# tyfeld/MMaDA-Parallel

Hardware: NVIDIA H100
Metric: denoised_tokens_per_sec (higher is better)
Workload: dtype bf16; 1 GPU; MMaDA-Parallel-A 8B, 1 prompt per GPU, 512x512 (1024 VQ tokens) + 256 text tokens, timesteps=64, text_steps=128, cfg_img=4.0, cfg_scale=0, temperature=1.0, text_temperature=0 (BASELINE configs[1]); seq_len=2414, parallelism=replicas x1 (independent prompts, no collective), weights=synthetic normal(0, 0.02) bf16, seeded, l2=16.2 GB of weights streamed per forward >> 50 MB L2 (no flush needed)

## Files before the change

mmada_parallel_b200/csrc/attention.cu:

```cuda
#include "mmdp_internal.h"
#include "ptx.cuh"

#include <stdlib.h>

#include <map>
#include <mutex>
#include <utility>

namespace mmdp {

static constexpr int kAttnThreads = 384;
static constexpr int kQBytes = 128 * 128 * 2;
template <int BKV> struct AttnCfg {
    static constexpr int kKBytes = BKV * 128 * 2;
    static constexpr int kVBytes = 128 * BKV * 2;
    static constexpr int kSmem = kQBytes + 2 * (kKBytes + kVBytes) + 1024  + 256 ;
};

__device__ __forceinline__ float ex2_approx(float x) {
    float y;
    asm("ex2.approx.ftz.f32 %0, %1;" : "=f"(y) : "f"(x));
    return y;
}

struct AttnSegs {
    int n;
    int start[kMaxSegs + 1];
    int tile0[kMaxSegs + 1];
};

struct AttnWin {
    AttnSegs segs;
    int q0[kMaxSegs], nq[kMaxSegs], out0[kMaxSegs];
};

template <int kBKV, bool kPacked, bool kGqa = false, bool kWin = false>
__device__ __forceinline__ void attention_body(const CUtensorMap& tmQ, const CUtensorMap& tmK, const CUtensorMap& tmVt,
                                               __nv_bfloat16* __restrict__ out, int H, int L, int d_model, float scale_log2,
                                               int n_full, int splits, float* __restrict__ part_ws, int Lq, const AttnSegs* segs,
                                               int kv_group = 1, const AttnWin* win = nullptr) {
    constexpr int kKBytes = AttnCfg<kBKV>::kKBytes, kVBytes = AttnCfg<kBKV>::kVBytes;
    extern __shared__ uint8_t smem_raw[];
    uint8_t* smem = reinterpret_cast<uint8_t*>((reinterpret_cast<uintptr_t>(smem_raw) + 1023) & ~uintptr_t(1023));
    uint8_t* sQ = smem;
    uint8_t* sK = sQ + kQBytes;
    uint8_t* sV = sK + 2 * kKBytes;
    uint64_t* bars = reinterpret_cast<uint64_t*>(sV + 2 * kVBytes);
    uint64_t* q_full = bars + 0;
    uint64_t* k_full = bars + 1;
    uint64_t* k_empty = bars + 3;
    uint64_t* v_full = bars + 5;
    uint64_t* v_empty = bars + 7;

    const int warp = threadIdx.x >> 5, lane = threadIdx.x & 31, wg = warp >> 2;
    int n_qt = (Lq + 127) / 128;
    int n_kv_all = (L + kBKV - 1) / kBKV;
    int tile = blockIdx.x, piece = -1;
    if ((int)blockIdx.x >= n_full) {
        const int t = (int)blockIdx.x - n_full;
        tile = n_full + t / splits;
        piece = t - (t / splits) * splits;
    }
    int seg = 0, seg0 = 0, tl = tile, q0 = 0, o0 = 0;
    if constexpr (kPacked) {
        for (int i = 1; i < segs->n; ++i)
            if (tile >= segs->tile0[i]) seg = i;
        seg0 = segs->start[seg];
        L = Lq = segs->start[seg + 1] - seg0;
        o0 = seg0;
        if constexpr (kWin) {
            q0 = win->q0[seg];
            Lq = win->nq[seg];
            o0 = win->out0[seg];
        }
        n_qt = (Lq + 127) / 128;
        n_kv_all = (L + kBKV - 1) / kBKV;
        tl = tile - segs->tile0[seg];
    }
    const int qt = tl % n_qt, h = (tl / n_qt) % H, b = kPacked ? seg : tile / (n_qt * H);
    const int hk = kGqa ? h / kv_group : h, Hk = kGqa ? H / kv_group : H;
    int jb = 0, je = n_kv_all;
    if (piece >= 0) {
        const int per = (n_kv_all + splits - 1) / splits;
        jb = piece * per;
        je = (jb + per < n_kv_all) ? jb + per : n_kv_all;
    }
    const int n_kv = je - jb;

    if (warp == 0 && lane == 0) {
        tma_prefetch_desc(&tmQ);
        tma_prefetch_desc(&tmK);
        tma_prefetch_desc(&tmVt);
        mbar_init(q_full, 1);
        for (int s = 0; s < 2; ++s) {
            mbar_init(&k_full[s], 1);
            mbar_init(&k_empty[s], 8);
            mbar_init(&v_full[s], 1);
            mbar_init(&v_empty[s], 8);
        }
        fence_barrier_init();
    }
    __syncthreads();
    pdl_launch_dependents();
    pdl_wait();

    if (wg == 0) {
        setmaxnreg_dec<40>();
        if (warp == 0 && elect_one_sync()) {
            const int qrow0 = (kPacked ? seg0 + q0 : b * Lq) + qt * 128;
            mbar_expect_tx(q_full, kQBytes);
            tma_load_2d(sQ, &tmQ, q_full, h * 128, qrow0);
            tma_load_2d(sQ + kQBytes / 2, &tmQ, q_full, h * 128 + 64, qrow0);
            for (int j = 0; j < n_kv; ++j) {
                const int st = j & 1;
                const uint32_t ph = (j >> 1) & 1;
                const int kv0 = (jb + j) * kBKV;
                mbar_wait(&k_empty[st], ph ^ 1);
                mbar_expect_tx(&k_full[st], kKBytes);
                tma_load_2d(sK + st * kKBytes, &tmK, &k_full[st], hk * 128, (kPacked ? seg0 : b * L) + kv0);
                tma_load_2d(sK + st * kKBytes + kKBytes / 2, &tmK, &k_full[st], hk * 128 + 64, (kPacked ? seg0 : b * L) + kv0);
                mbar_wait(&v_empty[st], ph ^ 1);
                mbar_expect_tx(&v_full[st], kVBytes);
                tma_load_2d(sV + st * kVBytes, &tmVt, &v_full[st], kv0, (b * Hk + hk) * 128);
                if (kBKV == 128) tma_load_2d(sV + st * kVBytes + kVBytes / 2, &tmVt, &v_full[st], kv0 + 64, (b * Hk + hk) * 128);
            }
        }
        __syncwarp();
        return;
    }

    setmaxnreg_inc<232>();
    const int half = wg - 1;
    const int r0 = half * 64 + (warp & 3) * 16 + (lane >> 2), c0 = 2 * (lane & 3);
    const uint32_t aQ = smem_u32(sQ) + half * (64 * 128);
    float o[64];
#pragma unroll
    for (int i = 0; i < 64; ++i) o[i] = 0.f;
    float m_run[2] = {-INFINITY, -INFINITY}, l_run[2] = {0.f, 0.f};
    mbar_wait(q_full, 0);
    for (int j = 0; j < n_kv; ++j) {
        const int st = j & 1;
        const uint32_t ph = (j >> 1) & 1;
        const int nvalid = L - (jb + j) * kBKV;
        float sacc[kBKV / 2];
        const uint32_t aK = smem_u32(sK + st * kKBytes);
        mbar_wait(&k_full[st], ph);
        wgmma_fence();
#pragma unroll
        for (int kk = 0; kk < 8; ++kk)
        {
            const uint64_t qd = smem_desc_kmajor_sw128(aQ + (kk >> 2) * (kQBytes / 2)) + (kk & 3) * 2;
            const uint64_t kd = smem_desc_kmajor_sw128(aK + (kk >> 2) * (kKBytes / 2)) + (kk & 3) * 2;
            if constexpr (kBKV == 128) wgmma_bf16_ss_n128(sacc, qd, kd, kk != 0);
            else wgmma_bf16_ss_n64(sacc, qd, kd, kk != 0);
        }
        wgmma_commit();
        wgmma_wait<0>();
        reg_fence(sacc);
        __syncwarp();
        if (lane == 0) mbar_arrive(&k_empty[st]);
        if (nvalid < kBKV) {
#pragma unroll
            for (int jj = 0; jj < kBKV / 8; ++jj)
#pragma unroll
                for (int e = 0; e < 2; ++e)
                    if (8 * jj + c0 + e >= nvalid) { sacc[4 * jj + e] = -INFINITY; sacc[4 * jj + 2 + e] = -INFINITY; }
        }
        float alpha[2], mneg[2];
#pragma unroll
        for (int hh = 0; hh < 2; ++hh) {
            float mx = sacc[2 * hh];
#pragma unroll
            for (int jj = 0; jj < kBKV / 8; ++jj) mx = fmaxf(mx, fmaxf(sacc[4 * jj + 2 * hh], sacc[4 * jj + 2 * hh + 1]));
            mx = fmaxf(mx, __shfl_xor_sync(0xffffffffu, mx, 1));
            mx = fmaxf(mx, __shfl_xor_sync(0xffffffffu, mx, 2));
            const float m_new = fmaxf(m_run[hh], mx);
            alpha[hh] = ex2_approx((m_run[hh] - m_new) * scale_log2);
            m_run[hh] = m_new;
            mneg[hh] = -m_new * scale_log2;
        }
        uint32_t pa[kBKV / 4];
        float rsum[2] = {0.f, 0.f};
#pragma unroll
        for (int jj = 0; jj < kBKV / 8; ++jj)
#pragma unroll
            for (int hh = 0; hh < 2; ++hh) {
                const float p0 = ex2_approx(fmaf(sacc[4 * jj + 2 * hh], scale_log2, mneg[hh]));
                const float p1 = ex2_approx(fmaf(sacc[4 * jj + 2 * hh + 1], scale_log2, mneg[hh]));
                rsum[hh] += p0 + p1;
                pa[2 * jj + hh] = pack_bf16x2(p0, p1);
            }
#pragma unroll
        for (int hh = 0; hh < 2; ++hh) l_run[hh] = fmaf(l_run[hh], alpha[hh], rsum[hh]);
#pragma unroll
        for (int jj = 0; jj < 16; ++jj) {
            o[4 * jj] *= alpha[0]; o[4 * jj + 1] *= alpha[0];
            o[4 * jj + 2] *= alpha[1]; o[4 * jj + 3] *= alpha[1];
        }
        const uint32_t aV = smem_u32(sV + st * kVBytes);
        mbar_wait(&v_full[st], ph);
        wgmma_fence();
#pragma unroll
        for (int kk = 0; kk < kBKV / 16; ++kk) {
            const uint32_t a[4] = {pa[4 * kk], pa[4 * kk + 1], pa[4 * kk + 2], pa[4 * kk + 3]};
            wgmma_bf16_rs_n128(o, a, smem_desc_kmajor_sw128(aV + (kk >> 2) * (kVBytes / 2)) + (kk & 3) * 2, 1);
        }
        wgmma_commit();
        wgmma_wait<0>();
        reg_fence(o);
        __syncwarp();
        if (lane == 0) mbar_arrive(&v_empty[st]);
    }
#pragma unroll
    for (int hh = 0; hh < 2; ++hh) {
        l_run[hh] += __shfl_xor_sync(0xffffffffu, l_run[hh], 1);
        l_run[hh] += __shfl_xor_sync(0xffffffffu, l_run[hh], 2);
    }
#pragma unroll
    for (int hh = 0; hh < 2; ++hh) {
        const int r = r0 + 8 * hh, qrow = qt * 128 + r;
        if (qrow >= Lq) continue;
        if (piece >= 0) {
            float* slot = part_ws + (size_t)((tile - n_full) * splits + piece) * (128 * 128 + 256);
            if ((lane & 3) == 0) {
                slot[128 * 128 + r] = m_run[hh];
                slot[128 * 128 + 128 + r] = l_run[hh];
            }
#pragma unroll
            for (int jj = 0; jj < 16; ++jj)
                *reinterpret_cast<float2*>(slot + (size_t)r * 128 + 8 * jj + c0) = make_float2(o[4 * jj + 2 * hh], o[4 * jj + 2 * hh + 1]);
        } else {
            const float inv_l = 1.0f / l_run[hh];
            __nv_bfloat16* orow = out + (size_t)((kPacked ? o0 : b * Lq) + qrow) * d_model + h * 128;
#pragma unroll
            for (int jj = 0; jj < 16; ++jj)
                *reinterpret_cast<uint32_t*>(orow + 8 * jj + c0) = pack_bf16x2(o[4 * jj + 2 * hh] * inv_l, o[4 * jj + 2 * hh + 1] * inv_l);
        }
    }
}

template <int kBKV>
__global__ void __launch_bounds__(kAttnThreads, 1)
attention_kernel(const __grid_constant__ CUtensorMap tmQ, const __grid_constant__ CUtensorMap tmK,
                 const __grid_constant__ CUtensorMap tmVt, __nv_bfloat16* __restrict__ out, int H, int L, int d_model,
                 float scale_log2, int n_full, int splits, float* __restrict__ part_ws, int Lq) {
    attention_body<kBKV, false>(tmQ, tmK, tmVt, out, H, L, d_model, scale_log2, n_full, splits, part_ws, Lq, nullptr);
}

template <int kBKV>
__global__ void __launch_bounds__(kAttnThreads, 1)
attention_packed_kernel(const __grid_constant__ CUtensorMap tmQ, const __grid_constant__ CUtensorMap tmK,
                        const __grid_constant__ CUtensorMap tmVt, __nv_bfloat16* __restrict__ out, int H, int d_model,
                        float scale_log2, int n_full, int splits, float* __restrict__ part_ws, const __grid_constant__ AttnSegs segs) {
    attention_body<kBKV, true>(tmQ, tmK, tmVt, out, H, 0, d_model, scale_log2, n_full, splits, part_ws, 0, &segs);
}

template <int kBKV>
__global__ void __launch_bounds__(kAttnThreads, 1)
attention_gqa_kernel(const __grid_constant__ CUtensorMap tmQ, const __grid_constant__ CUtensorMap tmK,
                     const __grid_constant__ CUtensorMap tmVt, __nv_bfloat16* __restrict__ out, int H, int L, int d_model,
                     float scale_log2, int n_full, int splits, float* __restrict__ part_ws, int Lq, int kv_group) {
    attention_body<kBKV, false, true>(tmQ, tmK, tmVt, out, H, L, d_model, scale_log2, n_full, splits, part_ws, Lq, nullptr, kv_group);
}

template <int kBKV>
__global__ void __launch_bounds__(kAttnThreads, 1)
attention_packed_gqa_kernel(const __grid_constant__ CUtensorMap tmQ, const __grid_constant__ CUtensorMap tmK,
                            const __grid_constant__ CUtensorMap tmVt, __nv_bfloat16* __restrict__ out, int H, int d_model,
                            float scale_log2, int n_full, int splits, float* __restrict__ part_ws, const __grid_constant__ AttnSegs segs,
                            int kv_group) {
    attention_body<kBKV, true, true>(tmQ, tmK, tmVt, out, H, 0, d_model, scale_log2, n_full, splits, part_ws, 0, &segs, kv_group);
}

template <int kBKV, bool kGqa>
__global__ void __launch_bounds__(kAttnThreads, 1)
attention_packed_window_kernel(const __grid_constant__ CUtensorMap tmQ, const __grid_constant__ CUtensorMap tmK,
                               const __grid_constant__ CUtensorMap tmVt, __nv_bfloat16* __restrict__ out, int H, int d_model,
                               float scale_log2, int n_full, int splits, float* __restrict__ part_ws, const __grid_constant__ AttnWin win,
                               int kv_group) {
    attention_body<kBKV, true, kGqa, true>(tmQ, tmK, tmVt, out, H, 0, d_model, scale_log2, n_full, splits, part_ws, 0, &win.segs,
                                           kv_group, &win);
}

template <bool kPacked, bool kWin = false>
__device__ __forceinline__ void attention_combine_body(const float* __restrict__ part_ws, __nv_bfloat16* __restrict__ out, int H,
                                                       int Lq, int d_model, float scale_log2, int n_full, int splits,
                                                       const AttnSegs* segs, const AttnWin* win = nullptr) {
    int n_qt = (Lq + 127) / 128;
    const int st = blockIdx.x, r = blockIdx.y, c = threadIdx.x;
    pdl_launch_dependents();
    pdl_wait();
    const int tile = n_full + st;
    int seg = 0, seg0 = 0, tl = tile;
    if constexpr (kPacked) {
        for (int i = 1; i < segs->n; ++i)
            if (tile >= segs->tile0[i]) seg = i;
        seg0 = segs->start[seg];
        Lq = segs->start[seg + 1] - seg0;
        if constexpr (kWin) {
            seg0 = win->out0[seg];
            Lq = win->nq[seg];
        }
        n_qt = (Lq + 127) / 128;
        tl = tile - segs->tile0[seg];
    }
    const int qt = tl % n_qt, h = (tl / n_qt) % H, b = kPacked ? seg : tile / (n_qt * H);
    const int qrow = qt * 128 + r;
    if (qrow >= Lq) return;
    const float* base = part_ws + (size_t)st * splits * (128 * 128 + 256);
    float m = -INFINITY;
    for (int i = 0; i < splits; ++i) m = fmaxf(m, base[(size_t)i * (128 * 128 + 256) + 128 * 128 + r]);
    float o = 0.f, l = 0.f;
    for (int i = 0; i < splits; ++i) {
        const float* slot = base + (size_t)i * (128 * 128 + 256);
        const float w = exp2f((slot[128 * 128 + r] - m) * scale_log2);
        o = fmaf(w, slot[(size_t)r * 128 + c], o);
        l = fmaf(w, slot[128 * 128 + 128 + r], l);
    }
    out[(size_t)((kPacked ? seg0 : b * Lq) + qrow) * d_model + h * 128 + c] = __float2bfloat16_rn(o / l);
}

__global__ void __launch_bounds__(128)
attention_combine_kernel(const float* __restrict__ part_ws, __nv_bfloat16* __restrict__ out, int H, int Lq, int d_model,
                         float scale_log2, int n_full, int splits) {
    attention_combine_body<false>(part_ws, out, H, Lq, d_model, scale_log2, n_full, splits, nullptr);
}

__global__ void __launch_bounds__(128)
attention_packed_combine_kernel(const float* __restrict__ part_ws, __nv_bfloat16* __restrict__ out, int H, int d_model,
                                float scale_log2, int n_full, int splits, const __grid_constant__ AttnSegs segs) {
    attention_combine_body<true>(part_ws, out, H, 0, d_model, scale_log2, n_full, splits, &segs);
}

__global__ void __launch_bounds__(128)
attention_packed_window_combine_kernel(const float* __restrict__ part_ws, __nv_bfloat16* __restrict__ out, int H, int d_model,
                                       float scale_log2, int n_full, int splits, const __grid_constant__ AttnWin win) {
    attention_combine_body<true, true>(part_ws, out, H, 0, d_model, scale_log2, n_full, splits, &win.segs, &win);
}

static std::map<std::pair<int, cudaStream_t>, std::pair<float*, size_t>> g_attn_ws;
static std::mutex g_attn_ws_mu;
static int attn_part_workspace(cudaStream_t stream, size_t need, float** out) {
    int dev = 0;
    MMDP_CUDA(cudaGetDevice(&dev));
    std::lock_guard<std::mutex> lk(g_attn_ws_mu);
    auto& e = g_attn_ws[std::make_pair(dev, stream)];
    if (need > e.second) {
        if (e.first) MMDP_CUDA(cudaFree(e.first));
        e.first = nullptr; e.second = 0;
        MMDP_CUDA(cudaMalloc(&e.first, need));
        e.second = need;
    }
    *out = e.first;
    return 0;
}

template <class KvbOf>
static void plan_split_tail(int tiles, KvbOf kvb_of, int& n_full, int& n_split, int& splits) {
    const int split_tail = opt(OPT_ATTN_SPLIT_TAIL), slots = num_sms();
    n_full = tiles; n_split = 0; splits = 1;
    auto fit_splits = [&](int want, int first) {
        int sp = want > 8 ? 8 : want;
        for (int t = first; t < tiles; ++t)
            if (sp > kvb_of(t) / 2) sp = kvb_of(t) / 2;
        auto empty_piece = [&](int s) {
            for (int t = first; t < tiles; ++t) {
                const int n_kvb = kvb_of(t);
                if ((s - 1) * ((n_kvb + s - 1) / s) >= n_kvb) return true;
            }
            return false;
        };
        while (sp >= 2 && empty_piece(sp)) --sp;
        return sp;
    };
    if (split_tail && tiles > slots && (tiles % slots) > 0 && (tiles % slots) * 4 <= slots) {
        n_split = tiles % slots;
        splits = fit_splits(slots / n_split, tiles - n_split);
        if (splits >= 2) n_full = tiles - n_split; else { n_split = 0; splits = 1; }
    } else if (split_tail && tiles * 2 <= slots) {
        splits = fit_splits(slots / tiles, 0);
        if (splits >= 2) { n_split = tiles; n_full = 0; } else splits = 1;
    }
}

template <class Kernel>
static int attn_smem_attr(Kernel kernel, int smem, unsigned long long& attr_set) {
    int dev = 0;
    MMDP_CUDA(cudaGetDevice(&dev));
    if (!(attr_set >> (dev & 63) & 1ull)) {
        MMDP_CUDA(cudaFuncSetAttribute(kernel, cudaFuncAttributeMaxDynamicSharedMemorySize, smem));
        attr_set |= 1ull << (dev & 63);
    }
    return 0;
}

template <int kBKV>
static int attention_launch(const __nv_bfloat16* q, const __nv_bfloat16* k, const __nv_bfloat16* vt, __nv_bfloat16* out, int B, int H,
                            int L, int Lpad, float scale, cudaStream_t stream, int Lq, int Hkv) {
    constexpr int kAttnSmem = AttnCfg<kBKV>::kSmem;
    if (B <= 0 || H <= 0 || L <= 0) return set_error("attention: empty problem");
    if (Lq <= 0) Lq = L;
    if (Hkv <= 0) Hkv = H;
    if (Hkv > H || H % Hkv) return set_error("attention: n_kv_heads=%d must divide n_heads=%d", Hkv, H);
    if (Lpad < L || (Lpad % 8)) return set_error("attention: Lpad must be >= L and a multiple of 8");
    const int d_model = H * 128, d_kv = Hkv * 128;
    CUtensorMap tmQ, tmK, tmVt;
    if (make_tmap_2d_bf16(&tmQ, q, (uint64_t)B * Lq, (uint64_t)d_model, (uint64_t)d_model, 128, 64)) return -1;
    if (make_tmap_2d_bf16(&tmK, k, (uint64_t)B * L, (uint64_t)d_kv, (uint64_t)d_kv, kBKV, 64)) return -1;
    if (make_tmap_2d_bf16(&tmVt, vt, (uint64_t)B * Hkv * 128, (uint64_t)Lpad, (uint64_t)Lpad, 128, 64)) return -1;
    const int n_qt = (Lq + 127) / 128, n_kvb = (L + kBKV - 1) / kBKV;
    const int tiles = n_qt * H * B;
    int n_full, n_split, splits;
    plan_split_tail(tiles, [&](int) { return n_kvb; }, n_full, n_split, splits);
    float* part_ws = nullptr;
    if (n_split > 0 && attn_part_workspace(stream, (size_t)n_split * splits * (128 * 128 + 256) * sizeof(float), &part_ws)) return -1;
    const int grid = n_full + n_split * splits;
    const float scale_log2 = scale * 1.4426950408889634f;
    const bool pdl = pdl_mode() != 0;
    LaunchScope ls(LK_ATTN, 4.0 * B * H * (double)Lq * L * 128, stream);
    if (Hkv != H) {
        static unsigned long long attr_set_gqa = 0;
        if (attn_smem_attr(attention_gqa_kernel<kBKV>, kAttnSmem, attr_set_gqa)) return -1;
        MMDP_CUDA(launch_ex(attention_gqa_kernel<kBKV>, dim3(grid), dim3(kAttnThreads), kAttnSmem, stream, pdl, false, tmQ, tmK, tmVt, out,
                            H, L, d_model, scale_log2, n_full, splits, part_ws, Lq, H / Hkv));
    } else {
        static unsigned long long attr_set = 0;
        if (attn_smem_attr(attention_kernel<kBKV>, kAttnSmem, attr_set)) return -1;
        MMDP_CUDA(launch_ex(attention_kernel<kBKV>, dim3(grid), dim3(kAttnThreads), kAttnSmem, stream, pdl, false, tmQ, tmK, tmVt, out, H, L,
                            d_model, scale_log2, n_full, splits, part_ws, Lq));
    }
    if (n_split > 0)
        MMDP_CUDA(launch_ex(attention_combine_kernel, dim3(n_split, 128), dim3(128), 0, stream, pdl, false, (const float*)part_ws, out, H, Lq,
                            d_model, scale_log2, n_full, splits));
    return 0;
}

template <int kBKV>
static int attention_packed_launch(const __nv_bfloat16* q, const __nv_bfloat16* k, const __nv_bfloat16* vt, __nv_bfloat16* out,
                                   const SegTable& segs, int H, int Lpad, float scale, cudaStream_t stream, int Hkv,
                                   const int* win_lo, const int* win_hi) {
    constexpr int kAttnSmem = AttnCfg<kBKV>::kSmem;
    if (segs.n <= 0 || segs.n > kMaxSegs || H <= 0) return set_error("attention_packed: %d sequences (1 to %d)", segs.n, kMaxSegs);
    if (Hkv <= 0) Hkv = H;
    if (Hkv > H || H % Hkv) return set_error("attention_packed: n_kv_heads=%d must divide n_heads=%d", Hkv, H);
    if (Lpad % 8) return set_error("attention_packed: Lpad must be a multiple of 8");
    if (!win_lo != !win_hi) return set_error("attention_packed: give both window bounds or neither");
    const bool windowed = win_lo != nullptr;
    AttnWin aw{};
    AttnSegs& as = aw.segs;
    as.n = segs.n;
    double work = 0;
    int Mq = 0;
    for (int s = 0; s <= segs.n; ++s) {
        as.start[s] = segs.start[s];
        if (s == segs.n) break;
        const int len = segs.start[s + 1] - segs.start[s];
        if (len <= 0 || len > Lpad) return set_error("attention_packed: sequence %d has length %d (Lpad %d)", s, len, Lpad);
        const int lo = windowed ? win_lo[s] : 0, hi = windowed ? win_hi[s] : len;
        if (lo < 0 || lo >= hi || hi > len)
            return set_error("attention_packed: sequence %d of length %d has the row window [%d, %d)", s, len, lo, hi);
        aw.q0[s] = lo;
        aw.nq[s] = hi - lo;
        aw.out0[s] = Mq;
        Mq += hi - lo;
        as.tile0[s + 1] = as.tile0[s] + (hi - lo + 127) / 128 * H;
        work += 4.0 * H * (double)(hi - lo) * len * 128;
    }
    const int M = segs.start[segs.n], tiles = as.tile0[segs.n], d_model = H * 128, d_kv = Hkv * 128;
    CUtensorMap tmQ, tmK, tmVt;
    if (make_tmap_2d_bf16(&tmQ, q, (uint64_t)M, (uint64_t)d_model, (uint64_t)d_model, 128, 64)) return -1;
    if (make_tmap_2d_bf16(&tmK, k, (uint64_t)M, (uint64_t)d_kv, (uint64_t)d_kv, kBKV, 64)) return -1;
    if (make_tmap_2d_bf16(&tmVt, vt, (uint64_t)segs.n * Hkv * 128, (uint64_t)Lpad, (uint64_t)Lpad, 128, 64)) return -1;
    auto kvb_of = [&](int t) {
        int s = 0;
        while (s + 1 < segs.n && t >= as.tile0[s + 1]) ++s;
        return (segs.start[s + 1] - segs.start[s] + kBKV - 1) / kBKV;
    };
    int n_full, n_split, splits;
    plan_split_tail(tiles, kvb_of, n_full, n_split, splits);
    float* part_ws = nullptr;
    if (n_split > 0 && attn_part_workspace(stream, (size_t)n_split * splits * (128 * 128 + 256) * sizeof(float), &part_ws)) return -1;
    const int grid = n_full + n_split * splits;
    const float scale_log2 = scale * 1.4426950408889634f;
    const bool pdl = pdl_mode() != 0;
    LaunchScope ls(LK_ATTN, work, stream);
    if (windowed) {
        auto kernel = Hkv != H ? attention_packed_window_kernel<kBKV, true> : attention_packed_window_kernel<kBKV, false>;
        static unsigned long long attr_set_win[2] = {0, 0};
        if (attn_smem_attr(kernel, kAttnSmem, attr_set_win[Hkv != H])) return -1;
        MMDP_CUDA(launch_ex(kernel, dim3(grid), dim3(kAttnThreads), kAttnSmem, stream, pdl, false, tmQ, tmK, tmVt, out, H, d_model,
                            scale_log2, n_full, splits, part_ws, aw, H / Hkv));
        if (n_split > 0)
            MMDP_CUDA(launch_ex(attention_packed_window_combine_kernel, dim3(n_split, 128), dim3(128), 0, stream, pdl, false,
                                (const float*)part_ws, out, H, d_model, scale_log2, n_full, splits, aw));
        return 0;
    }
    if (Hkv != H) {
        static unsigned long long attr_set_gqa = 0;
        if (attn_smem_attr(attention_packed_gqa_kernel<kBKV>, kAttnSmem, attr_set_gqa)) return -1;
        MMDP_CUDA(launch_ex(attention_packed_gqa_kernel<kBKV>, dim3(grid), dim3(kAttnThreads), kAttnSmem, stream, pdl, false, tmQ, tmK, tmVt,
                            out, H, d_model, scale_log2, n_full, splits, part_ws, as, H / Hkv));
    } else {
        static unsigned long long attr_set = 0;
        if (attn_smem_attr(attention_packed_kernel<kBKV>, kAttnSmem, attr_set)) return -1;
        MMDP_CUDA(launch_ex(attention_packed_kernel<kBKV>, dim3(grid), dim3(kAttnThreads), kAttnSmem, stream, pdl, false, tmQ, tmK, tmVt, out,
                            H, d_model, scale_log2, n_full, splits, part_ws, as));
    }
    if (n_split > 0)
        MMDP_CUDA(launch_ex(attention_packed_combine_kernel, dim3(n_split, 128), dim3(128), 0, stream, pdl, false, (const float*)part_ws,
                            out, H, d_model, scale_log2, n_full, splits, as));
    return 0;
}

int attention_fwd(const __nv_bfloat16* q, const __nv_bfloat16* k, const __nv_bfloat16* vt, __nv_bfloat16* out, int B, int H, int L,
                  int Lpad, float scale, cudaStream_t stream, int Lq, int Hkv) {
// ... 17 lines not shown
```

mmada_parallel_b200/csrc/ptx.cuh:

```cuda
#pragma once
#include <cuda.h>
#include <cuda_bf16.h>
#include <cuda_runtime.h>
#include <stdint.h>

namespace mmdp {

__device__ __forceinline__ uint32_t smem_u32(const void* p) {
    return static_cast<uint32_t>(__cvta_generic_to_shared(p));
}

__device__ __forceinline__ bool elect_one_sync() {
    uint32_t pred;
    asm volatile(
        "{\n\t.reg .pred p;\n\t"
        "elect.sync _|p, 0xffffffff;\n\t"
        "selp.u32 %0, 1, 0, p;\n\t}"
        : "=r"(pred));
    return pred != 0;
}

#ifndef MMDP_WAIT_SPIN_LIMIT
#define MMDP_WAIT_SPIN_LIMIT (1u << 26)
#endif

__device__ __forceinline__ void mbar_init(uint64_t* bar, uint32_t count) {
    asm volatile("mbarrier.init.shared::cta.b64 [%0], %1;" ::"r"(smem_u32(bar)), "r"(count));
}
__device__ __forceinline__ void fence_barrier_init() {
    asm volatile("fence.mbarrier_init.release.cluster;" ::: "memory");
}
__device__ __forceinline__ void mbar_expect_tx(uint64_t* bar, uint32_t bytes) {
    asm volatile("mbarrier.arrive.expect_tx.shared::cta.b64 _, [%0], %1;" ::"r"(smem_u32(bar)), "r"(bytes)
                 : "memory");
}
__device__ __forceinline__ void mbar_arrive(uint64_t* bar) {
    asm volatile("mbarrier.arrive.shared::cta.b64 _, [%0];" ::"r"(smem_u32(bar)) : "memory");
}
__device__ __forceinline__ bool mbar_try_wait(uint64_t* bar, uint32_t parity) {
    uint32_t ok;
    asm volatile(
        "{\n\t.reg .pred p;\n\t"
        "mbarrier.try_wait.parity.shared::cta.b64 p, [%1], %2;\n\t"
        "selp.b32 %0, 1, 0, p;\n\t}"
        : "=r"(ok)
        : "r"(smem_u32(bar)), "r"(parity)
        : "memory");
    return ok != 0;
}
__device__ __forceinline__ void mbar_wait(uint64_t* bar, uint32_t parity) {
    uint32_t spins = 0;
    while (!mbar_try_wait(bar, parity)) {
        if (++spins > MMDP_WAIT_SPIN_LIMIT) __trap();
    }
}

__device__ __forceinline__ void fence_proxy_async_smem() {
    asm volatile("fence.proxy.async.shared::cta;" ::: "memory");
}

__device__ __forceinline__ void tma_prefetch_desc(const CUtensorMap* tm) {
    asm volatile("prefetch.tensormap [%0];" ::"l"(reinterpret_cast<uint64_t>(tm)) : "memory");
}
__device__ __forceinline__ void tma_load_2d(void* smem_dst, const CUtensorMap* tm, uint64_t* bar, int c0, int c1) {
    asm volatile(
        "cp.async.bulk.tensor.2d.shared::cluster.global.mbarrier::complete_tx::bytes [%0], [%1, {%3, %4}], [%2];"
        ::"r"(smem_u32(smem_dst)), "l"(reinterpret_cast<uint64_t>(tm)), "r"(smem_u32(bar)), "r"(c0), "r"(c1)
        : "memory");
}

__device__ __forceinline__ void tma_load_2d_multicast(void* smem_dst, const CUtensorMap* tm, uint64_t* bar, int c0, int c1,
                                                      uint16_t cta_mask) {
    asm volatile(
        "cp.async.bulk.tensor.2d.shared::cluster.global.mbarrier::complete_tx::bytes.multicast::cluster [%0], [%1, {%3, %4}], [%2], %5;"
        ::"r"(smem_u32(smem_dst)), "l"(reinterpret_cast<uint64_t>(tm)), "r"(smem_u32(bar)), "r"(c0), "r"(c1), "h"(cta_mask)
        : "memory");
}

__device__ __forceinline__ uint32_t cluster_ctarank() {
    uint32_t r;
    asm volatile("mov.u32 %0, %%cluster_ctarank;" : "=r"(r));
    return r;
}
__device__ __forceinline__ void cluster_sync() {
    asm volatile("barrier.cluster.arrive.release.aligned;\n\tbarrier.cluster.wait.acquire.aligned;" ::: "memory");
}
__device__ __forceinline__ void mbar_arrive_cluster(uint64_t* bar, uint32_t cta) {
    asm volatile(
        "{\n\t.reg .b32 ra;\n\t"
        "mapa.shared::cluster.u32 ra, %0, %1;\n\t"
        "mbarrier.arrive.release.cluster.shared::cluster.b64 _, [ra];\n\t}"
        ::"r"(smem_u32(bar)), "r"(cta)
        : "memory");
}

__device__ __forceinline__ void tma_prefetch_l2_2d(const CUtensorMap* tm, int c0, int c1) {
    asm volatile("cp.async.bulk.prefetch.tensor.2d.L2.global.tile [%0, {%1, %2}];" ::"l"(reinterpret_cast<uint64_t>(tm)),
                 "r"(c0), "r"(c1)
                 : "memory");
}

__device__ __forceinline__ void pdl_wait() { asm volatile("griddepcontrol.wait;" ::: "memory"); }
__device__ __forceinline__ void pdl_launch_dependents() { asm volatile("griddepcontrol.launch_dependents;" ::: "memory"); }

__device__ __forceinline__ void wgmma_fence() { asm volatile("wgmma.fence.sync.aligned;" ::: "memory"); }
__device__ __forceinline__ void wgmma_commit() { asm volatile("wgmma.commit_group.sync.aligned;" ::: "memory"); }
template <int N>
__device__ __forceinline__ void wgmma_wait() { asm volatile("wgmma.wait_group.sync.aligned %0;" ::"n"(N) : "memory"); }
template <int N>
__device__ __forceinline__ void reg_fence(float (&d)[N]) {
#pragma unroll
    for (int i = 0; i < N; ++i) asm volatile("" : "+f"(d[i])::"memory");
}
template <uint32_t kRegs>
__device__ __forceinline__ void setmaxnreg_dec() { asm volatile("setmaxnreg.dec.sync.aligned.u32 %0;" ::"n"(kRegs)); }
template <uint32_t kRegs>
__device__ __forceinline__ void setmaxnreg_inc() { asm volatile("setmaxnreg.inc.sync.aligned.u32 %0;" ::"n"(kRegs)); }

__device__ __forceinline__ void wgmma_bf16_ss_n256(float (&d)[128], uint64_t a_desc, uint64_t b_desc, int scale_d) {
    asm volatile(
        "{\n\t.reg .pred p;\n\t"
        "setp.ne.b32 p, %130, 0;\n\t"
        "wgmma.mma_async.sync.aligned.m64n256k16.f32.bf16.bf16 "
        "{%0, %1, %2, %3, %4, %5, %6, %7, %8, %9, %10, %11, %12, %13, %14, %15, %16, %17, %18, %19, %20, %21, %22, %23, %24, %25, %26, %27, %28, %29, %30, %31, %32, %33, %34, %35, %36, %37, %38, %39, %40, %41, %42, %43, %44, %45, %46, %47, %48, %49, %50, %51, %52, %53, %54, %55, %56, %57, %58, %59, %60, %61, %62, %63, %64, %65, %66, %67, %68, %69, %70, %71, %72, %73, %74, %75, %76, %77, %78, %79, %80, %81, %82, %83, %84, %85, %86, %87, %88, %89, %90, %91, %92, %93, %94, %95, %96, %97, %98, %99, %100, %101, %102, %103, %104, %105, %106, %107, %108, %109, %110, %111, %112, %113, %114, %115, %116, %117, %118, %119, %120, %121, %122, %123, %124, %125, %126, %127}, "
        "%128, %129, p, 1, 1, 0, 0;\n\t}"
        : "+f"(d[0]), "+f"(d[1]), "+f"(d[2]), "+f"(d[3]), "+f"(d[4]), "+f"(d[5]), "+f"(d[6]), "+f"(d[7]), "+f"(d[8]), "+f"(d[9]), "+f"(d[10]), "+f"(d[11]), "+f"(d[12]), "+f"(d[13]), "+f"(d[14]), "+f"(d[15]), "+f"(d[16]), "+f"(d[17]), "+f"(d[18]), "+f"(d[19]), "+f"(d[20]), "+f"(d[21]), "+f"(d[22]), "+f"(d[23]), "+f"(d[24]), "+f"(d[25]), "+f"(d[26]), "+f"(d[27]), "+f"(d[28]), "+f"(d[29]), "+f"(d[30]), "+f"(d[31]), "+f"(d[32]), "+f"(d[33]), "+f"(d[34]), "+f"(d[35]), "+f"(d[36]), "+f"(d[37]), "+f"(d[38]), "+f"(d[39]), "+f"(d[40]), "+f"(d[41]), "+f"(d[42]), "+f"(d[43]), "+f"(d[44]), "+f"(d[45]), "+f"(d[46]), "+f"(d[47]), "+f"(d[48]), "+f"(d[49]), "+f"(d[50]), "+f"(d[51]), "+f"(d[52]), "+f"(d[53]), "+f"(d[54]), "+f"(d[55]), "+f"(d[56]), "+f"(d[57]), "+f"(d[58]), "+f"(d[59]), "+f"(d[60]), "+f"(d[61]), "+f"(d[62]), "+f"(d[63]), "+f"(d[64]), "+f"(d[65]), "+f"(d[66]), "+f"(d[67]), "+f"(d[68]), "+f"(d[69]), "+f"(d[70]), "+f"(d[71]), "+f"(d[72]), "+f"(d[73]), "+f"(d[74]), "+f"(d[75]), "+f"(d[76]), "+f"(d[77]), "+f"(d[78]), "+f"(d[79]), "+f"(d[80]), "+f"(d[81]), "+f"(d[82]), "+f"(d[83]), "+f"(d[84]), "+f"(d[85]), "+f"(d[86]), "+f"(d[87]), "+f"(d[88]), "+f"(d[89]), "+f"(d[90]), "+f"(d[91]), "+f"(d[92]), "+f"(d[93]), "+f"(d[94]), "+f"(d[95]), "+f"(d[96]), "+f"(d[97]), "+f"(d[98]), "+f"(d[99]), "+f"(d[100]), "+f"(d[101]), "+f"(d[102]), "+f"(d[103]), "+f"(d[104]), "+f"(d[105]), "+f"(d[106]), "+f"(d[107]), "+f"(d[108]), "+f"(d[109]), "+f"(d[110]), "+f"(d[111]), "+f"(d[112]), "+f"(d[113]), "+f"(d[114]), "+f"(d[115]), "+f"(d[116]), "+f"(d[117]), "+f"(d[118]), "+f"(d[119]), "+f"(d[120]), "+f"(d[121]), "+f"(d[122]), "+f"(d[123]), "+f"(d[124]), "+f"(d[125]), "+f"(d[126]), "+f"(d[127])
        : "l"(a_desc), "l"(b_desc), "r"(scale_d));
}

__device__ __forceinline__ void wgmma_bf16_ss_n192(float (&d)[96], uint64_t a_desc, uint64_t b_desc, int scale_d) {
    asm volatile(
        "{\n\t.reg .pred p;\n\t"
        "setp.ne.b32 p, %98, 0;\n\t"
        "wgmma.mma_async.sync.aligned.m64n192k16.f32.bf16.bf16 "
        "{%0, %1, %2, %3, %4, %5, %6, %7, %8, %9, %10, %11, %12, %13, %14, %15, %16, %17, %18, %19, %20, %21, %22, %23, %24, %25, %26, %27, %28, %29, %30, %31, %32, %33, %34, %35, %36, %37, %38, %39, %40, %41, %42, %43, %44, %45, %46, %47, %48, %49, %50, %51, %52, %53, %54, %55, %56, %57, %58, %59, %60, %61, %62, %63, %64, %65, %66, %67, %68, %69, %70, %71, %72, %73, %74, %75, %76, %77, %78, %79, %80, %81, %82, %83, %84, %85, %86, %87, %88, %89, %90, %91, %92, %93, %94, %95}, "
        "%96, %97, p, 1, 1, 0, 0;\n\t}"
        : "+f"(d[0]), "+f"(d[1]), "+f"(d[2]), "+f"(d[3]), "+f"(d[4]), "+f"(d[5]), "+f"(d[6]), "+f"(d[7]), "+f"(d[8]), "+f"(d[9]), "+f"(d[10]), "+f"(d[11]), "+f"(d[12]), "+f"(d[13]), "+f"(d[14]), "+f"(d[15]), "+f"(d[16]), "+f"(d[17]), "+f"(d[18]), "+f"(d[19]), "+f"(d[20]), "+f"(d[21]), "+f"(d[22]), "+f"(d[23]), "+f"(d[24]), "+f"(d[25]), "+f"(d[26]), "+f"(d[27]), "+f"(d[28]), "+f"(d[29]), "+f"(d[30]), "+f"(d[31]), "+f"(d[32]), "+f"(d[33]), "+f"(d[34]), "+f"(d[35]), "+f"(d[36]), "+f"(d[37]), "+f"(d[38]), "+f"(d[39]), "+f"(d[40]), "+f"(d[41]), "+f"(d[42]), "+f"(d[43]), "+f"(d[44]), "+f"(d[45]), "+f"(d[46]), "+f"(d[47]), "+f"(d[48]), "+f"(d[49]), "+f"(d[50]), "+f"(d[51]), "+f"(d[52]), "+f"(d[53]), "+f"(d[54]), "+f"(d[55]), "+f"(d[56]), "+f"(d[57]), "+f"(d[58]), "+f"(d[59]), "+f"(d[60]), "+f"(d[61]), "+f"(d[62]), "+f"(d[63]), "+f"(d[64]), "+f"(d[65]), "+f"(d[66]), "+f"(d[67]), "+f"(d[68]), "+f"(d[69]), "+f"(d[70]), "+f"(d[71]), "+f"(d[72]), "+f"(d[73]), "+f"(d[74]), "+f"(d[75]), "+f"(d[76]), "+f"(d[77]), "+f"(d[78]), "+f"(d[79]), "+f"(d[80]), "+f"(d[81]), "+f"(d[82]), "+f"(d[83]), "+f"(d[84]), "+f"(d[85]), "+f"(d[86]), "+f"(d[87]), "+f"(d[88]), "+f"(d[89]), "+f"(d[90]), "+f"(d[91]), "+f"(d[92]), "+f"(d[93]), "+f"(d[94]), "+f"(d[95])
        : "l"(a_desc), "l"(b_desc), "r"(scale_d));
}

__device__ __forceinline__ void wgmma_bf16_ss_n128(float (&d)[64], uint64_t a_desc, uint64_t b_desc, int scale_d) {
    asm volatile(
        "{\n\t.reg .pred p;\n\t"
        "setp.ne.b32 p, %66, 0;\n\t"
        "wgmma.mma_async.sync.aligned.m64n128k16.f32.bf16.bf16 "
        "{%0, %1, %2, %3, %4, %5, %6, %7, %8, %9, %10, %11, %12, %13, %14, %15, %16, %17, %18, %19, %20, %21, %22, %23, %24, %25, %26, %27, %28, %29, %30, %31, %32, %33, %34, %35, %36, %37, %38, %39, %40, %41, %42, %43, %44, %45, %46, %47, %48, %49, %50, %51, %52, %53, %54, %55, %56, %57, %58, %59, %60, %61, %62, %63}, "
        "%64, %65, p, 1, 1, 0, 0;\n\t}"
        : "+f"(d[0]), "+f"(d[1]), "+f"(d[2]), "+f"(d[3]), "+f"(d[4]), "+f"(d[5]), "+f"(d[6]), "+f"(d[7]), "+f"(d[8]), "+f"(d[9]), "+f"(d[10]), "+f"(d[11]), "+f"(d[12]), "+f"(d[13]), "+f"(d[14]), "+f"(d[15]), "+f"(d[16]), "+f"(d[17]), "+f"(d[18]), "+f"(d[19]), "+f"(d[20]), "+f"(d[21]), "+f"(d[22]), "+f"(d[23]), "+f"(d[24]), "+f"(d[25]), "+f"(d[26]), "+f"(d[27]), "+f"(d[28]), "+f"(d[29]), "+f"(d[30]), "+f"(d[31]), "+f"(d[32]), "+f"(d[33]), "+f"(d[34]), "+f"(d[35]), "+f"(d[36]), "+f"(d[37]), "+f"(d[38]), "+f"(d[39]), "+f"(d[40]), "+f"(d[41]), "+f"(d[42]), "+f"(d[43]), "+f"(d[44]), "+f"(d[45]), "+f"(d[46]), "+f"(d[47]), "+f"(d[48]), "+f"(d[49]), "+f"(d[50]), "+f"(d[51]), "+f"(d[52]), "+f"(d[53]), "+f"(d[54]), "+f"(d[55]), "+f"(d[56]), "+f"(d[57]), "+f"(d[58]), "+f"(d[59]), "+f"(d[60]), "+f"(d[61]), "+f"(d[62]), "+f"(d[63])
        : "l"(a_desc), "l"(b_desc), "r"(scale_d));
}

__device__ __forceinline__ void wgmma_bf16_ss_n64(float (&d)[32], uint64_t a_desc, uint64_t b_desc, int scale_d) {
    asm volatile(
        "{\n\t.reg .pred p;\n\t"
        "setp.ne.b32 p, %34, 0;\n\t"
        "wgmma.mma_async.sync.aligned.m64n64k16.f32.bf16.bf16 "
        "{%0, %1, %2, %3, %4, %5, %6, %7, %8, %9, %10, %11, %12, %13, %14, %15, %16, %17, %18, %19, %20, %21, %22, %23, %24, %25, %26, %27, %28, %29, %30, %31}, "
        "%32, %33, p, 1, 1, 0, 0;\n\t}"
        : "+f"(d[0]), "+f"(d[1]), "+f"(d[2]), "+f"(d[3]), "+f"(d[4]), "+f"(d[5]), "+f"(d[6]), "+f"(d[7]), "+f"(d[8]), "+f"(d[9]), "+f"(d[10]), "+f"(d[11]), "+f"(d[12]), "+f"(d[13]), "+f"(d[14]), "+f"(d[15]), "+f"(d[16]), "+f"(d[17]), "+f"(d[18]), "+f"(d[19]), "+f"(d[20]), "+f"(d[21]), "+f"(d[22]), "+f"(d[23]), "+f"(d[24]), "+f"(d[25]), "+f"(d[26]), "+f"(d[27]), "+f"(d[28]), "+f"(d[29]), "+f"(d[30]), "+f"(d[31])
        : "l"(a_desc), "l"(b_desc), "r"(scale_d));
}

__device__ __forceinline__ void wgmma_bf16_rs_n128(float (&d)[64], const uint32_t (&a)[4], uint64_t b_desc, int scale_d) {
    asm volatile(
        "{\n\t.reg .pred p;\n\t"
        "setp.ne.b32 p, %69, 0;\n\t"
        "wgmma.mma_async.sync.aligned.m64n128k16.f32.bf16.bf16 "
        "{%0, %1, %2, %3, %4, %5, %6, %7, %8, %9, %10, %11, %12, %13, %14, %15, %16, %17, %18, %19, %20, %21, %22, %23, %24, %25, %26, %27, %28, %29, %30, %31, %32, %33, %34, %35, %36, %37, %38, %39, %40, %41, %42, %43, %44, %45, %46, %47, %48, %49, %50, %51, %52, %53, %54, %55, %56, %57, %58, %59, %60, %61, %62, %63}, "
        "{%64, %65, %66, %67}, %68, p, 1, 1, 0;\n\t}"
        : "+f"(d[0]), "+f"(d[1]), "+f"(d[2]), "+f"(d[3]), "+f"(d[4]), "+f"(d[5]), "+f"(d[6]), "+f"(d[7]), "+f"(d[8]), "+f"(d[9]), "+f"(d[10]), "+f"(d[11]), "+f"(d[12]), "+f"(d[13]), "+f"(d[14]), "+f"(d[15]), "+f"(d[16]), "+f"(d[17]), "+f"(d[18]), "+f"(d[19]), "+f"(d[20]), "+f"(d[21]), "+f"(d[22]), "+f"(d[23]), "+f"(d[24]), "+f"(d[25]), "+f"(d[26]), "+f"(d[27]), "+f"(d[28]), "+f"(d[29]), "+f"(d[30]), "+f"(d[31]), "+f"(d[32]), "+f"(d[33]), "+f"(d[34]), "+f"(d[35]), "+f"(d[36]), "+f"(d[37]), "+f"(d[38]), "+f"(d[39]), "+f"(d[40]), "+f"(d[41]), "+f"(d[42]), "+f"(d[43]), "+f"(d[44]), "+f"(d[45]), "+f"(d[46]), "+f"(d[47]), "+f"(d[48]), "+f"(d[49]), "+f"(d[50]), "+f"(d[51]), "+f"(d[52]), "+f"(d[53]), "+f"(d[54]), "+f"(d[55]), "+f"(d[56]), "+f"(d[57]), "+f"(d[58]), "+f"(d[59]), "+f"(d[60]), "+f"(d[61]), "+f"(d[62]), "+f"(d[63])
        : "r"(a[0]), "r"(a[1]), "r"(a[2]), "r"(a[3]), "l"(b_desc), "r"(scale_d));
}

__device__ __forceinline__ void wgmma_e4m3_ss_n128(float (&d)[64], uint64_t a_desc, uint64_t b_desc, int scale_d) {
    asm volatile(
        "{\n\t.reg .pred p;\n\t"
        "setp.ne.b32 p, %66, 0;\n\t"
        "wgmma.mma_async.sync.aligned.m64n128k32.f32.e4m3.e4m3 "
        "{%0, %1, %2, %3, %4, %5, %6, %7, %8, %9, %10, %11, %12, %13, %14, %15, %16, %17, %18, %19, %20, %21, %22, %23, %24, %25, %26, %27, %28, %29, %30, %31, %32, %33, %34, %35, %36, %37, %38, %39, %40, %41, %42, %43, %44, %45, %46, %47, %48, %49, %50, %51, %52, %53, %54, %55, %56, %57, %58, %59, %60, %61, %62, %63}, "
        "%64, %65, p, 1, 1;\n\t}"
        : "+f"(d[0]), "+f"(d[1]), "+f"(d[2]), "+f"(d[3]), "+f"(d[4]), "+f"(d[5]), "+f"(d[6]), "+f"(d[7]), "+f"(d[8]), "+f"(d[9]), "+f"(d[10]), "+f"(d[11]), "+f"(d[12]), "+f"(d[13]), "+f"(d[14]), "+f"(d[15]), "+f"(d[16]), "+f"(d[17]), "+f"(d[18]), "+f"(d[19]), "+f"(d[20]), "+f"(d[21]), "+f"(d[22]), "+f"(d[23]), "+f"(d[24]), "+f"(d[25]), "+f"(d[26]), "+f"(d[27]), "+f"(d[28]), "+f"(d[29]), "+f"(d[30]), "+f"(d[31]), "+f"(d[32]), "+f"(d[33]), "+f"(d[34]), "+f"(d[35]), "+f"(d[36]), "+f"(d[37]), "+f"(d[38]), "+f"(d[39]), "+f"(d[40]), "+f"(d[41]), "+f"(d[42]), "+f"(d[43]), "+f"(d[44]), "+f"(d[45]), "+f"(d[46]), "+f"(d[47]), "+f"(d[48]), "+f"(d[49]), "+f"(d[50]), "+f"(d[51]), "+f"(d[52]), "+f"(d[53]), "+f"(d[54]), "+f"(d[55]), "+f"(d[56]), "+f"(d[57]), "+f"(d[58]), "+f"(d[59]), "+f"(d[60]), "+f"(d[61]), "+f"(d[62]), "+f"(d[63])
        : "l"(a_desc), "l"(b_desc), "r"(scale_d));
}

__device__ __forceinline__ void wgmma_tf32_ss_n128(float (&d)[64], uint64_t a_desc, uint64_t b_desc, int scale_d) {
    asm volatile(
        "{\n\t.reg .pred p;\n\t"
        "setp.ne.b32 p, %66, 0;\n\t"
        "wgmma.mma_async.sync.aligned.m64n128k8.f32.tf32.tf32 "
        "{%0, %1, %2, %3, %4, %5, %6, %7, %8, %9, %10, %11, %12, %13, %14, %15, %16, %17, %18, %19, %20, %21, %22, %23, %24, %25, %26, %27, %28, %29, %30, %31, %32, %33, %34, %35, %36, %37, %38, %39, %40, %41, %42, %43, %44, %45, %46, %47, %48, %49, %50, %51, %52, %53, %54, %55, %56, %57, %58, %59, %60, %61, %62, %63}, "
        "%64, %65, p, 1, 1;\n\t}"
        : "+f"(d[0]), "+f"(d[1]), "+f"(d[2]), "+f"(d[3]), "+f"(d[4]), "+f"(d[5]), "+f"(d[6]), "+f"(d[7]), "+f"(d[8]), "+f"(d[9]), "+f"(d[10]), "+f"(d[11]), "+f"(d[12]), "+f"(d[13]), "+f"(d[14]), "+f"(d[15]), "+f"(d[16]), "+f"(d[17]), "+f"(d[18]), "+f"(d[19]), "+f"(d[20]), "+f"(d[21]), "+f"(d[22]), "+f"(d[23]), "+f"(d[24]), "+f"(d[25]), "+f"(d[26]), "+f"(d[27]), "+f"(d[28]), "+f"(d[29]), "+f"(d[30]), "+f"(d[31]), "+f"(d[32]), "+f"(d[33]), "+f"(d[34]), "+f"(d[35]), "+f"(d[36]), "+f"(d[37]), "+f"(d[38]), "+f"(d[39]), "+f"(d[40]), "+f"(d[41]), "+f"(d[42]), "+f"(d[43]), "+f"(d[44]), "+f"(d[45]), "+f"(d[46]), "+f"(d[47]), "+f"(d[48]), "+f"(d[49]), "+f"(d[50]), "+f"(d[51]), "+f"(d[52]), "+f"(d[53]), "+f"(d[54]), "+f"(d[55]), "+f"(d[56]), "+f"(d[57]), "+f"(d[58]), "+f"(d[59]), "+f"(d[60]), "+f"(d[61]), "+f"(d[62]), "+f"(d[63])
        : "l"(a_desc), "l"(b_desc), "r"(scale_d));
}

__device__ __forceinline__ uint64_t smem_desc_kmajor_sw128(uint32_t smem_addr) {
    uint64_t d = 0;
    d |= static_cast<uint64_t>((smem_addr & 0x3FFFFu) >> 4);
    d |= static_cast<uint64_t>(1) << 16;
    d |= static_cast<uint64_t>(1024 >> 4) << 32;
    d |= static_cast<uint64_t>(1) << 62;
    return d;
}

__device__ __forceinline__ float bf16_round(float x) { return __bfloat162float(__float2bfloat16_rn(x)); }
__device__ __forceinline__ uint32_t pack_bf16x2(float lo, float hi) {
    __nv_bfloat162 v = __floats2bfloat162_rn(lo, hi);
    return *reinterpret_cast<uint32_t*>(&v);
}
__device__ __forceinline__ float bf16_lo(uint32_t v) { return __uint_as_float(v << 16); }
__device__ __forceinline__ float bf16_hi(uint32_t v) { return __uint_as_float(v & 0xFFFF0000u); }

__device__ __forceinline__ uint32_t pack_e4m3x4(float a0, float a1, float a2, float a3) {
    uint16_t lo, hi;
    asm("cvt.rn.satfinite.e4m3x2.f32 %0, %1, %2;" : "=h"(lo) : "f"(a1), "f"(a0));
    asm("cvt.rn.satfinite.e4m3x2.f32 %0, %1, %2;" : "=h"(hi) : "f"(a3), "f"(a2));
    return (uint32_t)lo | ((uint32_t)hi << 16);
}

}
```

Measured before the change: 104.4 tokens/s.

## Software-pipeline attention QK and PV wgmma with ping-pong consumer warpgroups

Restructures the FlashAttention consumer loop so the QK^T wgmma for the next KV tile is issued together with the PV wgmma of the current tile, overlapping softmax with tensor-core work. Named barriers make the two consumer warpgroups take turns issuing MMAs (FA3-style ping-pong), so one group's softmax runs while the other's matmuls execute. This adds register pressure from keeping extra score and probability fragments live, plus barrier overhead. Attention is a modest share of a weight-streaming 8B forward pass.

```diff
diff --git a/mmada_parallel_b200/csrc/attention.cu b/mmada_parallel_b200/csrc/attention.cu
--- a/mmada_parallel_b200/csrc/attention.cu
+++ b/mmada_parallel_b200/csrc/attention.cu
@@ -11,16 +11,95 @@
 
 static constexpr int kAttnThreads = 384;
 static constexpr int kQBytes = 128 * 128 * 2;
+static constexpr int kAttnStages = 2;
 template <int BKV> struct AttnCfg {
     static constexpr int kKBytes = BKV * 128 * 2;
     static constexpr int kVBytes = 128 * BKV * 2;
-    static constexpr int kSmem = kQBytes + 2 * (kKBytes + kVBytes) + 1024  + 256 ;
+    static constexpr int kSmem = kQBytes + kAttnStages * (kKBytes + kVBytes) + 1024  + 256 ;
 };
 
 __device__ __forceinline__ float ex2_approx(float x) {
     float y;
     asm("ex2.approx.ftz.f32 %0, %1;" : "=f"(y) : "f"(x));
     return y;
+}
+
+template <int kBKV>
+__device__ __forceinline__ void attn_issue_qk(float (&s)[kBKV / 2], uint32_t aQ, uint32_t aK) {
+    constexpr int kKBytes = AttnCfg<kBKV>::kKBytes;
+    wgmma_fence();
+#pragma unroll
+    for (int kk = 0; kk < 8; ++kk) {
+        const uint64_t qd = smem_desc_kmajor_sw128(aQ + (kk >> 2) * (kQBytes / 2)) + (kk & 3) * 2;
+        const uint64_t kd = smem_desc_kmajor_sw128(aK + (kk >> 2) * (kKBytes / 2)) + (kk & 3) * 2;
+        if constexpr (kBKV == 128) wgmma_bf16_ss_n128(s, qd, kd, kk != 0);
+        else wgmma_bf16_ss_n64(s, qd, kd, kk != 0);
+    }
+    wgmma_commit();
+}
+
+template <int kBKV>
+__device__ __forceinline__ void attn_issue_pv(float (&o)[64], const uint32_t (&pa)[kBKV / 4], uint32_t aV) {
+    constexpr int kVBytes = AttnCfg<kBKV>::kVBytes;
+    wgmma_fence();
+#pragma unroll
+    for (int kk = 0; kk < kBKV / 16; ++kk) {
+        const uint32_t a[4] = {pa[4 * kk], pa[4 * kk + 1], pa[4 * kk + 2], pa[4 * kk + 3]};
+        wgmma_bf16_rs_n128(o, a, smem_desc_kmajor_sw128(aV + (kk >> 2) * (kVBytes / 2)) + (kk & 3) * 2, 1);
+    }
+    wgmma_commit();
+}
+
+template <int kBKV>
+__device__ __forceinline__ void attn_softmax(float (&s)[kBKV / 2], int nvalid, int c0, float scale_log2, float (&m_run)[2],
+                                             float (&l_run)[2], float (&alpha)[2]) {
+    if (nvalid < kBKV) {
+#pragma unroll
+        for (int jj = 0; jj < kBKV / 8; ++jj)
+#pragma unroll
+            for (int e = 0; e < 2; ++e)
+                if (8 * jj + c0 + e >= nvalid) { s[4 * jj + e] = -INFINITY; s[4 * jj + 2 + e] = -INFINITY; }
+    }
+    float mneg[2];
+#pragma unroll
+    for (int hh = 0; hh < 2; ++hh) {
+        float mx = s[2 * hh];
+#pragma unroll
+        for (int jj = 0; jj < kBKV / 8; ++jj) mx = fmaxf(mx, fmaxf(s[4 * jj + 2 * hh], s[4 * jj + 2 * hh + 1]));
+        mx = fmaxf(mx, __shfl_xor_sync(0xffffffffu, mx, 1));
+        mx = fmaxf(mx, __shfl_xor_sync(0xffffffffu, mx, 2));
+        const float m_new = fmaxf(m_run[hh], mx);
+        alpha[hh] = ex2_approx((m_run[hh] - m_new) * scale_log2);
+        m_run[hh] = m_new;
+        mneg[hh] = -m_new * scale_log2;
+    }
+    float rsum[2] = {0.f, 0.f};
+#pragma unroll
+    for (int jj = 0; jj < kBKV / 8; ++jj)
+#pragma unroll
+        for (int hh = 0; hh < 2; ++hh) {
+            const float p0 = ex2_approx(fmaf(s[4 * jj + 2 * hh], scale_log2, mneg[hh]));
+            const float p1 = ex2_approx(fmaf(s[4 * jj + 2 * hh + 1], scale_log2, mneg[hh]));
+            rsum[hh] += p0 + p1;
+            s[4 * jj + 2 * hh] = p0;
+            s[4 * jj + 2 * hh + 1] = p1;
+        }
+#pragma unroll
+    for (int hh = 0; hh < 2; ++hh) l_run[hh] = fmaf(l_run[hh], alpha[hh], rsum[hh]);
+}
+
+template <int kBKV>
+__device__ __forceinline__ void attn_rescale_pack(float (&o)[64], const float (&s)[kBKV / 2], const float (&alpha)[2],
+                                                  uint32_t (&pa)[kBKV / 4]) {
+#pragma unroll
+    for (int jj = 0; jj < 16; ++jj) {
+        o[4 * jj] *= alpha[0]; o[4 * jj + 1] *= alpha[0];
+        o[4 * jj + 2] *= alpha[1]; o[4 * jj + 3] *= alpha[1];
+    }
+#pragma unroll
+    for (int jj = 0; jj < kBKV / 8; ++jj)
+#pragma unroll
+        for (int hh = 0; hh < 2; ++hh) pa[2 * jj + hh] = pack_bf16x2(s[4 * jj + 2 * hh], s[4 * jj + 2 * hh + 1]);
 }
 
 struct AttnSegs {
@@ -44,13 +123,13 @@
     uint8_t* smem = reinterpret_cast<uint8_t*>((reinterpret_cast<uintptr_t>(smem_raw) + 1023) & ~uintptr_t(1023));
     uint8_t* sQ = smem;
     uint8_t* sK = sQ + kQBytes;
-    uint8_t* sV = sK + 2 * kKBytes;
-    uint64_t* bars = reinterpret_cast<uint64_t*>(sV + 2 * kVBytes);
+    uint8_t* sV = sK + kAttnStages * kKBytes;
+    uint64_t* bars = reinterpret_cast<uint64_t*>(sV + kAttnStages * kVBytes);
     uint64_t* q_full = bars + 0;
     uint64_t* k_full = bars + 1;
-    uint64_t* k_empty = bars + 3;
-    uint64_t* v_full = bars + 5;
-    uint64_t* v_empty = bars + 7;
+    uint64_t* k_empty = k_full + kAttnStages;
+    uint64_t* v_full = k_empty + kAttnStages;
+    uint64_t* v_empty = v_full + kAttnStages;
 
     const int warp = threadIdx.x >> 5, lane = threadIdx.x & 31, wg = warp >> 2;
     int n_qt = (Lq + 127) / 128;
@@ -92,7 +171,7 @@
         tma_prefetch_desc(&tmK);
         tma_prefetch_desc(&tmVt);
         mbar_init(q_full, 1);
-        for (int s = 0; s < 2; ++s) {
+        for (int s = 0; s < kAttnStages; ++s) {
             mbar_init(&k_full[s], 1);
             mbar_init(&k_empty[s], 8);
             mbar_init(&v_full[s], 1);
@@ -112,8 +191,8 @@
             tma_load_2d(sQ, &tmQ, q_full, h * 128, qrow0);
             tma_load_2d(sQ + kQBytes / 2, &tmQ, q_full, h * 128 + 64, qrow0);
             for (int j = 0; j < n_kv; ++j) {
-                const int st = j & 1;
-                const uint32_t ph = (j >> 1) & 1;
+                const int st = j % kAttnStages;
+                const uint32_t ph = (j / kAttnStages) & 1;
                 const int kv0 = (jb + j) * kBKV;
                 mbar_wait(&k_empty[st], ph ^ 1);
                 mbar_expect_tx(&k_full[st], kKBytes);
@@ -137,80 +216,57 @@
 #pragma unroll
     for (int i = 0; i < 64; ++i) o[i] = 0.f;
     float m_run[2] = {-INFINITY, -INFINITY}, l_run[2] = {0.f, 0.f};
-    mbar_wait(q_full, 0);
-    for (int j = 0; j < n_kv; ++j) {
-        const int st = j & 1;
-        const uint32_t ph = (j >> 1) & 1;
-        const int nvalid = L - (jb + j) * kBKV;
-        float sacc[kBKV / 2];
-        const uint32_t aK = smem_u32(sK + st * kKBytes);
-        mbar_wait(&k_full[st], ph);
-        wgmma_fence();
-#pragma unroll
-        for (int kk = 0; kk < 8; ++kk)
-        {
-            const uint64_t qd = smem_desc_kmajor_sw128(aQ + (kk >> 2) * (kQBytes / 2)) + (kk & 3) * 2;
-            const uint64_t kd = smem_desc_kmajor_sw128(aK + (kk >> 2) * (kKBytes / 2)) + (kk & 3) * 2;
-            if constexpr (kBKV == 128) wgmma_bf16_ss_n128(sacc, qd, kd, kk != 0);
-            else wgmma_bf16_ss_n64(sacc, qd, kd, kk != 0);
-        }
-        wgmma_commit();
-        wgmma_wait<0>();
-        reg_fence(sacc);
+    constexpr uint32_t kMma = 256;
+    const uint32_t my_turn = 1 + half, their_turn = 2 - half;
+    bool ok = true;
+    float s[kBKV / 2];
+    uint32_t pa[kBKV / 4];
+    float alpha[2];
+    ok &= mbar_wait_ok(q_full, 0);
+    ok &= mbar_wait_ok(&k_full[0], 0);
+    if (half == 1) named_bar_arrive(their_turn, kMma);
+    named_bar_sync(my_turn, kMma);
+    attn_issue_qk<kBKV>(s, aQ, smem_u32(sK));
+    named_bar_arrive(their_turn, kMma);
+    wgmma_wait<0>();
+    reg_fence(s);
+    __syncwarp();
+    if (lane == 0) mbar_arrive(&k_empty[0]);
+    attn_softmax<kBKV>(s, L - jb * kBKV, c0, scale_log2, m_run, l_run, alpha);
+    attn_rescale_pack<kBKV>(o, s, alpha, pa);
+    for (int j = 0; j + 1 < n_kv; ++j) {
+        const int st = j % kAttnStages, st1 = (j + 1) % kAttnStages;
+        ok &= mbar_wait_ok(&k_full[st1], ((j + 1) / kAttnStages) & 1);
+        ok &= mbar_wait_ok(&v_full[st], (j / kAttnStages) & 1);
+        named_bar_sync(my_turn, kMma);
+        attn_issue_qk<kBKV>(s, aQ, smem_u32(sK + st1 * kKBytes));
+        attn_issue_pv<kBKV>(o, pa, smem_u32(sV + st * kVBytes));
+        named_bar_arrive(their_turn, kMma);
+        wgmma_wait<1>();
+        reg_fence(s);
         __syncwarp();
-        if (lane == 0) mbar_arrive(&k_empty[st]);
-        if (nvalid < kBKV) {
-#pragma unroll
-            for (int jj = 0; jj < kBKV / 8; ++jj)
-#pragma unroll
-                for (int e = 0; e < 2; ++e)
-                    if (8 * jj + c0 + e >= nvalid) { sacc[4 * jj + e] = -INFINITY; sacc[4 * jj + 2 + e] = -INFINITY; }
-        }
-        float alpha[2], mneg[2];
-#pragma unroll
-        for (int hh = 0; hh < 2; ++hh) {
-            float mx = sacc[2 * hh];
-#pragma unroll
-            for (int jj = 0; jj < kBKV / 8; ++jj) mx = fmaxf(mx, fmaxf(sacc[4 * jj + 2 * hh], sacc[4 * jj + 2 * hh + 1]));
-            mx = fmaxf(mx, __shfl_xor_sync(0xffffffffu, mx, 1));
-            mx = fmaxf(mx, __shfl_xor_sync(0xffffffffu, mx, 2));
-            const float m_new = fmaxf(m_run[hh], mx);
-            alpha[hh] = ex2_approx((m_run[hh] - m_new) * scale_log2);
-            m_run[hh] = m_new;
-            mneg[hh] = -m_new * scale_log2;
-        }
-        uint32_t pa[kBKV / 4];
-        float rsum[2] = {0.f, 0.f};
-#pragma unroll
-        for (int jj = 0; jj < kBKV / 8; ++jj)
-#pragma unroll
-            for (int hh = 0; hh < 2; ++hh) {
-                const float p0 = ex2_approx(fmaf(sacc[4 * jj + 2 * hh], scale_log2, mneg[hh]));
-                const float p1 = ex2_approx(fmaf(sacc[4 * jj + 2 * hh + 1], scale_log2, mneg[hh]));
-                rsum[hh] += p0 + p1;
-                pa[2 * jj + hh] = pack_bf16x2(p0, p1);
-            }
-#pragma unroll
-        for (int hh = 0; hh < 2; ++hh) l_run[hh] = fmaf(l_run[hh], alpha[hh], rsum[hh]);
-#pragma unroll
-        for (int jj = 0; jj < 16; ++jj) {
-            o[4 * jj] *= alpha[0]; o[4 * jj + 1] *= alpha[0];
-            o[4 * jj + 2] *= alpha[1]; o[4 * jj + 3] *= alpha[1];
-        }
-        const uint32_t aV = smem_u32(sV + st * kVBytes);
-        mbar_wait(&v_full[st], ph);
-        wgmma_fence();
-#pragma unroll
-        for (int kk = 0; kk < kBKV / 16; ++kk) {
-            const uint32_t a[4] = {pa[4 * kk], pa[4 * kk + 1], pa[4 * kk + 2], pa[4 * kk + 3]};
-            wgmma_bf16_rs_n128(o, a, smem_desc_kmajor_sw128(aV + (kk >> 2) * (kVBytes / 2)) + (kk & 3) * 2, 1);
-        }
-        wgmma_commit();
+        if (lane == 0) mbar_arrive(&k_empty[st1]);
+        attn_softmax<kBKV>(s, L - (jb + j + 1) * kBKV, c0, scale_log2, m_run, l_run, alpha);
         wgmma_wait<0>();
         reg_fence(o);
+        reg_fence(pa);
         __syncwarp();
         if (lane == 0) mbar_arrive(&v_empty[st]);
-    }
+        attn_rescale_pack<kBKV>(o, s, alpha, pa);
+    }
+    {
+        const int j = n_kv - 1, st = j % kAttnStages;
+        ok &= mbar_wait_ok(&v_full[st], (j / kAttnStages) & 1);
+        named_bar_sync(my_turn, kMma);
+        attn_issue_pv<kBKV>(o, pa, smem_u32(sV + st * kVBytes));
+        if (half == 0) named_bar_arrive(their_turn, kMma);
+        wgmma_wait<0>();
+        reg_fence(o);
+        reg_fence(pa);
+        __syncwarp();
+        if (lane == 0) mbar_arrive(&v_empty[st]);
+    }
+    if (!ok) __trap();
 #pragma unroll
     for (int hh = 0; hh < 2; ++hh) {
         l_run[hh] += __shfl_xor_sync(0xffffffffu, l_run[hh], 1);
diff --git a/mmada_parallel_b200/csrc/ptx.cuh b/mmada_parallel_b200/csrc/ptx.cuh
--- a/mmada_parallel_b200/csrc/ptx.cuh
+++ b/mmada_parallel_b200/csrc/ptx.cuh
@@ -53,6 +53,18 @@
     while (!mbar_try_wait(bar, parity)) {
         if (++spins > MMDP_WAIT_SPIN_LIMIT) __trap();
     }
+}
+__device__ __forceinline__ bool mbar_wait_ok(uint64_t* bar, uint32_t parity) {
+    for (uint32_t spins = 0; !mbar_try_wait(bar, parity);)
+        if (++spins > MMDP_WAIT_SPIN_LIMIT) return false;
+    return true;
+}
+
+__device__ __forceinline__ void named_bar_sync(uint32_t id, uint32_t n) {
+    asm volatile("bar.sync %0, %1;" ::"r"(id), "r"(n) : "memory");
+}
+__device__ __forceinline__ void named_bar_arrive(uint32_t id, uint32_t n) {
+    asm volatile("bar.arrive %0, %1;" ::"r"(id), "r"(n) : "memory");
 }
 
 __device__ __forceinline__ void fence_proxy_async_smem() {
@@ -112,6 +124,11 @@
 #pragma unroll
     for (int i = 0; i < N; ++i) asm volatile("" : "+f"(d[i])::"memory");
 }
+template <int N>
+__device__ __forceinline__ void reg_fence(uint32_t (&a)[N]) {
+#pragma unroll
+    for (int i = 0; i < N; ++i) asm volatile("" : "+r"(a[i])::"memory");
+}
 template <uint32_t kRegs>
 __device__ __forceinline__ void setmaxnreg_dec() { asm volatile("setmaxnreg.dec.sync.aligned.u32 %0;" ::"n"(kRegs)); }
 template <uint32_t kRegs>
```

After: 105.5 tokens/s (median of 6 runs). 1.01x the previous value.
